# kazuto1011/dusty-gan

Measured on AMD Instinct MI355X. Metric: G+D train images/sec on 64x1024 LiDAR (steps/sec beside it), higher is better.
Workload: dtype bf16

## Files before the change

dusty_gan_amd/_lib.py:

```python
import ctypes as C
import os
import subprocess

_HERE = os.path.dirname(os.path.abspath(__file__))
CSRC = os.path.join(_HERE, "csrc")
LIB_PATH = os.path.join(CSRC, "libdustygan_hip.so")
if os.environ.get("DUSTY_GAN_LIB_DIAG"):
    _d = os.environ["DUSTY_GAN_LIB_DIAG"]
    LIB_PATH = os.path.join(CSRC, "libdustygan_hip_diag%s.so" % ("" if _d == "1" else _d))

DG_OK, DG_EINVAL, DG_EUNSUPPORTED, DG_EHIP = 0, 1, 2, 3
DG_F32, DG_BF16 = 0, 1
DG_BF16X2 = 2
MODE_S2, MODE_UP, MODE_GEMM = 0, 1, 2
EPI_LINEAR, EPI_LRELU, EPI_MASK = 0, 1, 2
DG_FORCE_AUTO, DG_FORCE_DIRECT, DG_FORCE_MFMA, DG_FORCE_THIN, DG_FORCE_LOCKSTEP, DG_FORCE_PINGPONG = 0, 1, 2, 3, 4, 5
DG_FORCE_WG_REGSTAGED, DG_FORCE_WG_DMA_PAIRS, DG_FORCE_WG_DMA_NOPAIRS, DG_FORCE_PINGPONG_SINGLE, DG_FORCE_PROJ_STREAM = 6, 7, 8, 9, 10
DG_FORCE_FP32X3 = 0x100
DG_CONV_FAMILY_DIRECT, DG_CONV_FAMILY_MFMA, DG_CONV_FAMILY_THIN, DG_CONV_FAMILY_LOCKSTEP, DG_CONV_FAMILY_PINGPONG = 1, 2, 3, 4, 5
DG_CONV_FAMILY_PROJ_STREAM = 6
DG_WGRAD_VARIANT_DIRECT, DG_WGRAD_VARIANT_MFMA, DG_WGRAD_VARIANT_THIN, DG_WGRAD_VARIANT_DMA, DG_WGRAD_VARIANT_THIN_MFMA = 1, 2, 3, 5, 7
POLICY_BITS = {"brightness": 1, "saturation": 2, "contrast": 4, "translation": 8, "cutout": 16}

_ERR = {1: "DG_EINVAL (bad argument)", 2: "DG_EUNSUPPORTED (shape not supported by the requested kernel)",
# ... 181 lines not shown
    "dg_transpose_shadow_multi_frags": [_P, _P, _I, _I, _I, C.POINTER(DgUpFrag), _I, _P],
    "dg_transpose_shadow_multi_tail": [_P, _P, _I, _I, _I, C.POINTER(DgUpFrag), _I, _P, _P, _I, _I, _P, _I, _P, _I, _P],
    "dg_philox_bits": [_U64, _U64, _U64, _L, _P, _P],
    "dg_philox_fill": [_U64, _U64, _U64, _I, _F, _F, _I, _I, _L, _P, _P],
    "dg_aug_draw": [_U64, _U64, _U64, _I, _I, _I, _P, _P, _P],
    "dg_counter_add": [_P, _U64, _P],
    "dg_step_prologue": [_P, _P, _I, C.POINTER(DgDraw), _I, _P],
    "dg_step_prologue_fetch": [_P, _P, _I, C.POINTER(DgDraw), _I, C.POINTER(DgFetch), _P],
    "dg_counter_add_multi": [_P, _P, _I, _P],
    "dg_counter_add_multi_snap": [_P, _P, _I, _I, _P, _I, _P, _I, _P],
    "dg_philox_fill_dev": [_U64, _U64, _P, _I, _F, _F, _I, _I, _L, _P, _P],
    "dg_aug_draw_dev": [_U64, _U64, _P, _I, _I, _I, _P, _P, _P],
    "dg_philox_logistic_dev": [_U64, _U64, _P, _F, _L, _P, _P],
    "dg_adam_ema_step_dev": [_P, _P, _P, _P, _P, _P, _I, _L, _F, _F, _F, _F, _F, _P, _F, _P],
    "dg_adam_fused": [_P, _P, _P, _P, _P, _I, C.POINTER(DgOptSeg), _I, _F, _F, _F, _F, _P, _F, _P],
    "dg_adam_proj_fused": [_P, _P, _P, _P, _I, _P, _P, _I, _I, _L, _I, _F, _F, _F, _F, _F, _P, _F, _P],
    "dg_inv_loss_grad": [_P, _L, _I, _P, _P, _P, _I, _I, _L, _F, _P, _I, _P, _I, _P, _P, _I, _P, _P],
    "dg_inv_loss_grad_add": [_P, _L, _I, _P, _P, _P, _I, _I, _L, _F, _P, _I, _P, _I, _P, _P, _I, _P, _P],
    "dg_inv_chamfer_scatter": [_P, _P, _I, _L, _P, _P],
    "dg_inv_chamfer_grad": [_P, _P, _P, _P, _P, _P, _P, _P, _P, _P, _P, _I, _F, _F, _F, _F, _F, _I, _L, _F, _F, _I, _P, _I, _P,
                            _I, _P, _P, _I, _P, _P],
    "dg_sphere_adam": [_P, _L, _L, _P, _P, _P, _P, _P, _P, _P, _I, _I, _I, _P, _I, _F, _F, _F, _I, _U64, _U64, _I, _P],
    "dg_depth_metrics": [_P, _P, _P, _P, _I, _I, _F, _I, _L, _F, _F, _P, _P],
    "dg_feat_compose": [_P, _P, _P, _I, _I, _I, _I, _I, _P],
    "dg_feat_compose_bwd": [_P, _P, _P, _P, _P, _P, _P, _I, _I, _I, _I, _I, _I, _P],
    "dg_alpha_adam": [_P, _P, _P, _P, _P, _P, _I, _F, _F, _F, _L, _P],
    "dg_corrupt_mask": [_P, _P, _P, _P, _F, _I, _I, _I, _P, _P],
    "dg_additive_noise": [_P, _P, _F, _L, _P, _P],
    "dg_median3x3": [_P, _I, _I, _I, _P, _P],
    "dg_hole_fill": [_P, _P, _I, _I, _I, _F, _P, _P, _P],
# ... 287 lines not shown
```

dusty_gan_amd/csrc/optim.hip:

```cpp
#include "adam.h"
#include "step_inputs.h"
#include "thin_up_frag.h"
#include <cstdlib>
typedef __attribute__((ext_vector_type(4))) float f32x4_opt;

template <typename T>
__global__ __launch_bounds__(256) void adam_ema_kernel(float* __restrict__ p, const float* __restrict__ grad,
                                                       float* __restrict__ m, float* __restrict__ v,
                                                       float* __restrict__ ema, T* __restrict__ shadow, long n4,
                                                       float gscale, float lr_bc1, float inv_sqrt_bc2, float b1,
                                                       float b2, float eps, float ema_decay,
                                                       const unsigned long long* __restrict__ stepp, float lr) {
  if (stepp) {
    const float t = adam_step_t(stepp);
    lr_bc1 = adam_lr_bc1(lr, b1, t);
    inv_sqrt_bc2 = adam_inv_sqrt_bc2(b2, t);
  }
  const AdamCoef c{lr_bc1, inv_sqrt_bc2, b2, eps, ema_decay};
  for (long i = (long)blockIdx.x * blockDim.x + threadIdx.x; i < n4; i += (long)gridDim.x * blockDim.x) {
    const float4 g4 = ((const float4*)grad)[i];
    const float4 v4 = ((const float4*)v)[i];
    float4 p4 = ((const float4*)p)[i];
    float4 m4 = m ? ((const float4*)m)[i] : make_float4(0.f, 0.f, 0.f, 0.f);
    float4 e4 = ema ? ((const float4*)ema)[i] : make_float4(0.f, 0.f, 0.f, 0.f);
// ... 5 lines not shown
      mv[k] = b1 * mv[k] + (1.f - b1) * gg[k];
      adam_ema_apply(mv[k], gg[k], vv[k], pv[k], ev[k], c);
    }
    ((float4*)p)[i] = make_float4(pv[0], pv[1], pv[2], pv[3]);
    ((float4*)v)[i] = make_float4(vv[0], vv[1], vv[2], vv[3]);
    if (m) ((float4*)m)[i] = make_float4(mv[0], mv[1], mv[2], mv[3]);
    if (ema) ((float4*)ema)[i] = make_float4(ev[0], ev[1], ev[2], ev[3]);
    if (shadow) shadow_store4(shadow + 4 * i, 0, pv);
  }
}

typedef DgOptSeg OptSeg;
#define OPT_MAX_SEG DG_OPT_MAX_SEG
struct OptSegs { OptSeg s[OPT_MAX_SEG]; int n; int total_blocks; };

template <typename ST>
__global__ __launch_bounds__(256) void adam_fused_kernel(float* __restrict__ p, float* __restrict__ grad, float* __restrict__ v,
                                                         float* __restrict__ ema, ST* __restrict__ shadow, OptSegs segs,
                                                         float gscale, float lr, float b2, float eps, float ema_decay,
                                                         const unsigned long long* __restrict__ stepp) {
  __shared__ f32x4_opt s_part[16][17];
  __shared__ float tile[16 * 65 > 8 * 129 ? 16 * 65 : 8 * 129];
  int k = 0;
  for (int i = 1; i < segs.n; ++i)
    if ((int)blockIdx.x >= segs.s[i].first_block) k = i;
  const OptSeg& sg = segs.s[k];
  const int blk = (int)blockIdx.x - sg.first_block;
  const AdamCoef c{lr, adam_inv_sqrt_bc2(b2, adam_step_t(stepp)), b2, eps, ema_decay};
  struct State { float4 v4, p4, e4; f32x4_opt g0; };
  auto state_load = [&](long i4, bool acc) {
    State st;
    st.v4 = ((const float4*)v)[i4];
    st.p4 = ((const float4*)p)[i4];
    st.e4 = ema ? ((const float4*)ema)[i4] : make_float4(0.f, 0.f, 0.f, 0.f);
    st.g0 = acc ? ((const f32x4_opt*)grad)[i4] : f32x4_opt{0.f, 0.f, 0.f, 0.f};
    return st;
  };
  auto update4 = [&](long i4, f32x4_opt g, const State& st, float (&pn)[4]) {
    const float4 v4 = st.v4, p4 = st.p4, e4 = st.e4;
    ((f32x4_opt*)grad)[i4] = g;
    const float gg[4] = {g[0] * gscale, g[1] * gscale, g[2] * gscale, g[3] * gscale};
    float vv[4] = {v4.x, v4.y, v4.z, v4.w}, ev[4] = {e4.x, e4.y, e4.z, e4.w};
    pn[0] = p4.x; pn[1] = p4.y; pn[2] = p4.z; pn[3] = p4.w;
#pragma unroll
    for (int q = 0; q < 4; ++q) adam_ema_apply(gg[q], gg[q], vv[q], pn[q], ev[q], c);
    ((float4*)p)[i4] = make_float4(pn[0], pn[1], pn[2], pn[3]);
    ((float4*)v)[i4] = make_float4(vv[0], vv[1], vv[2], vv[3]);
    if (ema) ((float4*)ema)[i4] = make_float4(ev[0], ev[1], ev[2], ev[3]);
    if (shadow) shadow_store4(shadow, 4 * i4, pn);
  };
  auto part_sum = [&](long e4, int sp0, int step) {
    f32x4_opt acc = {0.f, 0.f, 0.f, 0.f};
    const f32x4_opt* src = (const f32x4_opt*)sg.part + e4;
    const long stride = sg.numel / 4;
    int sp = sp0;
    for (; sp + 7 * step < sg.splits; sp += 8 * step) {
      f32x4_opt r[8];
#pragma unroll
      for (int j = 0; j < 8; ++j) r[j] = __builtin_nontemporal_load(src + (long)(sp + j * step) * stride);
#pragma unroll
      for (int j = 0; j < 8; ++j) acc += r[j];
// ... 70 lines not shown
  g += st.g0;
  float pn[4];
  update4(i4, g, st, pn);
  float* tl = (float*)tile;
#pragma unroll
  for (int q = 0; q < 4; ++q) tl[ty * (CW + 1) + 4 * tx + q] = pn[q];
  __syncthreads();
  for (int c = threadIdx.x; c < CW; c += 256) {
    ST* dst = (ST*)sg.shadow_t + ((long)tap * Co + co0 + c) * Ci + ci0;
    for (int r0 = 0; r0 < R; r0 += 4) {
      const float o[4] = {tl[(r0 + 0) * (CW + 1) + c], tl[(r0 + 1) * (CW + 1) + c], tl[(r0 + 2) * (CW + 1) + c],
                          tl[(r0 + 3) * (CW + 1) + c]};
      shadow_store4(dst, r0, o);
    }
  }
}

typedef __attribute__((ext_vector_type(2))) __bf16 ad_bf16x2;
#define APF_ROWS 64

template <typename ST>
__global__ __launch_bounds__(256) void adam_proj_fused_kernel(float* __restrict__ p, float* __restrict__ v,
                                                              float* __restrict__ ema, ST* __restrict__ shadow,
                                                              const bf16* __restrict__ dp0, const bf16* __restrict__ zT,
                                                              int nb, long Np, int K, float wscale, float gscale, float lr,
                                                              float b2, float eps, float ema_decay,
                                                              const unsigned long long* __restrict__ stepp) {
  extern __shared__ __attribute__((aligned(16))) unsigned char smem[];
  const int nbp = nb / 2;
  unsigned* z2 = (unsigned*)smem;
// ... 49 lines not shown
  const int tx = threadIdx.x & 31, ty = threadIdx.x >> 5;
  const float* src = master + (long)tap * Ci * Co;
  T* dst = shadow + (long)tap * Ci * Co;
  for (int r = ty; r < 32; r += 8) {
    const int ci = ci0 + r, co = co0 + tx;
    tile[r][tx] = (ci < Ci && co < Co) ? src[(long)ci * Co + co] : 0.f;
  }
  __syncthreads();
  for (int r = ty; r < 32; r += 8) {
    const int co = co0 + r, ci = ci0 + tx;
    if (ci < Ci && co < Co) dst[(long)co * Ci + ci] = (T)tile[tx][r];
  }
}

struct UpFrags { DgUpFrag f[4]; int n; int first_block; };
template <typename T>
__global__ __launch_bounds__(256) void transpose_shadow_multi_kernel(const float* __restrict__ master,
                                                                     const long long* __restrict__ desc, int nseg,
                                                                     UpFrags uf, CounterAdds ca, int ca_block) {
  if ((int)blockIdx.x == ca_block) { counter_adds_body(ca); return; }
  if (uf.n > 0 && (int)blockIdx.x >= uf.first_block) {
    const int job = (int)blockIdx.x - uf.first_block, per = 3 * UP_FRAG_BLOCKS;
    const DgUpFrag& f = uf.f[job / per];
    const int cls = (job % per) / UP_FRAG_BLOCKS, e = ((job % per) % UP_FRAG_BLOCKS) * 256 + threadIdx.x;
    const float* w = master + f.off;
    up_frag_element(cls, e, f.N, f.Hc, f.adj,
                    [&](int tap, int n, int k) { return (float)(bf16)w[tap * f.m_st + n * f.m_sn + k * f.m_sk]; },
                    (unsigned char*)f.frag);
    return;
  }
  int sidx = 0;
  for (int i = 1; i < nseg; ++i)
    if ((long long)blockIdx.x >= desc[5 * i + 4]) sidx = i;
  const long long* d = desc + 5 * sidx;
  const int Ci = (int)d[2], Co = (int)d[3];
  const int tci = (Ci + 31) / 32, tco = (Co + 31) / 32;
  int t = (int)(blockIdx.x - d[4]);
  const int tap = t / (tci * tco);
  t -= tap * tci * tco;
  const int ti = t / tco, tj = t % tco;
  transpose_tile32(master + d[0], (T*)d[1], Ci, Co, tap, ti, tj);
}

template <typename T>
__global__ void cast_kernel(const float* __restrict__ src, T* __restrict__ dst, long n) {
  const long i = (long)blockIdx.x * blockDim.x + threadIdx.x;
  if (i < n) dst[i] = (T)src[i];
}

struct CastItems { const float* src[16]; void* dst[16]; long first8[17]; int n; };
__device__ __forceinline__ void x2_pack8(const float* __restrict__ src, unsigned short* __restrict__ dst, long i8) {
  const float4 a = ((const float4*)src)[2 * i8], b = ((const float4*)src)[2 * i8 + 1];
  const float v[8] = {a.x, a.y, a.z, a.w, b.x, b.y, b.z, b.w};
  unsigned hi[4], lo[4];
#pragma unroll
  for (int e = 0; e < 4; ++e) {
    const bf16 h0 = (bf16)v[2 * e], h1 = (bf16)v[2 * e + 1];
    const bf16 l0 = (bf16)(v[2 * e] - (float)h0), l1 = (bf16)(v[2 * e + 1] - (float)h1);
// ... 113 lines not shown
  if (dtype == DG_BF16) cast_kernel<bf16><<<nblk(n), 256, 0, s>>>(src, (bf16*)dst, n);
  else cast_kernel<float><<<nblk(n), 256, 0, s>>>(src, (float*)dst, n);
  HIP_CHECK_RET(hipGetLastError());
  return DG_OK;
}

int dg_transpose_shadow(const float* master, void* dst, int dtype, int Ci, int Co, void* s_) {
  hipStream_t s = (hipStream_t)s_;
  dim3 grid((Co + 31) / 32, (Ci + 31) / 32, 16);
  if (dtype == DG_BF16) transpose_shadow_kernel<bf16><<<grid, 256, 0, s>>>(master, (bf16*)dst, Ci, Co);
  else transpose_shadow_kernel<float><<<grid, 256, 0, s>>>(master, (float*)dst, Ci, Co);
  HIP_CHECK_RET(hipGetLastError());
  return DG_OK;
}

int dg_adam_fused(float* p, float* grad, float* v, float* ema, void* shadow, int shadow_dtype, const DgOptSeg* segs, int nseg,
                  float gscale, float lr, float beta2, float eps, const unsigned long long* step_dev, float ema_decay, void* s_) {
  hipStream_t s = (hipStream_t)s_;
  if (!p || !grad || !v || !segs || !step_dev || nseg < 1 || nseg > DG_OPT_MAX_SEG) return DG_EINVAL;
  if (shadow && shadow_dtype != DG_BF16 && shadow_dtype != DG_F32) return DG_EINVAL;
  if ((((size_t)p | (size_t)grad | (size_t)v | (size_t)ema | (size_t)shadow) & 15) != 0) return DG_EINVAL;
  OptSegs g{};
  long blocks = 0;
  for (int i = 0; i < nseg; ++i) {
    DgOptSeg q = segs[i];
    if (q.off < 0 || q.numel <= 0 || q.off % 4 != 0 || q.numel % 4 != 0 || q.splits < 0 || (q.splits > 0) != (q.part != nullptr))
      return DG_EINVAL;
    if (q.part && ((size_t)q.part & 15) != 0) return DG_EINVAL;
    if (q.kind == 1) {
      if (q.ci <= 0 || q.co <= 0 || !(q.co == 64 || q.co % 128 == 0) || q.ci % 16 != 0 || q.numel != 16LL * q.ci * q.co ||
          !q.shadow_t || !shadow || ((size_t)q.shadow_t & 15) != 0 || q.ws_src)
        return DG_EINVAL;
      q.first_block = (int)blocks;
      blocks += q.numel / 1024;
    } else if (q.kind == 0) {
      if (q.ws_src && (q.ws_n < 1 || q.ws_stride < q.numel || ((size_t)q.ws_src & 15) != 0 || q.ws_stride % 4 != 0)) return DG_EINVAL;
      if (q.splits > 64) {
        if (q.ws_src) return DG_EINVAL;
        q.kind = 2;
        q.first_block = (int)blocks;
        blocks += (q.numel / 4 + 15) / 16;
      } else {
        q.first_block = (int)blocks;
        blocks += (q.numel / 4 + 255) / 256;
      }
    } else {
      return DG_EINVAL;
    }
    if (blocks > (1L << 30)) return DG_EUNSUPPORTED;
    g.s[i] = q;
  }
  g.n = nseg;
  g.total_blocks = (int)blocks;
  if (shadow && shadow_dtype == DG_BF16)
    adam_fused_kernel<bf16><<<(unsigned)blocks, 256, 0, s>>>(p, grad, v, ema, (bf16*)shadow, g, gscale, lr, beta2, eps, ema_decay, step_dev);
  else
    adam_fused_kernel<float><<<(unsigned)blocks, 256, 0, s>>>(p, grad, v, ema, (float*)shadow, g, gscale, lr, beta2, eps, ema_decay, step_dev);
  HIP_CHECK_RET(hipGetLastError());
  return DG_OK;
}

int dg_adam_proj_fused(float* p, float* v, float* ema, void* shadow, int shadow_dtype, const void* dp0, const void* zT,
                       int op_dtype, int nb, long Np, int K, float wscale, float gscale, float lr, float beta2,
                       float eps, const unsigned long long* step_dev, float ema_decay, void* s_) {
  hipStream_t s = (hipStream_t)s_;
  if (!p || !v || !dp0 || !zT || !step_dev) return DG_EINVAL;
  const int x3 = (op_dtype & DG_FORCE_FP32X3) ? 1 : 0;
  op_dtype &= ~DG_FORCE_FP32X3;
  if ((op_dtype != DG_BF16 && op_dtype != DG_F32) || (x3 && op_dtype != DG_F32) || Np <= 0 || nb < 2) return DG_EUNSUPPORTED;
  const size_t lds = ((size_t)(nb / 2) * K + (size_t)APF_ROWS * (nb / 2)) * 4;
  const bool valu_ok = nb <= 64 && nb % 2 == 0 && K % 4 == 0 && K / 4 <= 256 && 256 % (K / 4) == 0 && lds <= 64 * 1024;
  const bool mfma_ok = Np % 128 == 0 && K % 128 == 0;
  if (op_dtype == DG_F32 && !mfma_ok) return DG_EUNSUPPORTED;
  if (!valu_ok || mfma_ok) {
// ... 67 lines not shown
```

dusty_gan_amd/csrc/step_inputs.h:

```cpp
#pragma once
#include "common.h"

struct CounterAdds {
  unsigned long long* c[8]; unsigned long long d[8]; int k;
  int snap_idx, snap_n, snap_ring; const float* snap_src; float* snap_dst;
};
__device__ __forceinline__ void counter_adds_body(const CounterAdds& a) {
  if ((int)threadIdx.x >= a.k) return;
  const unsigned long long v = *a.c[threadIdx.x];
  *a.c[threadIdx.x] = v + a.d[threadIdx.x];
  if ((int)threadIdx.x == a.snap_idx) {
    float* dst = a.snap_dst + (long)(v % (unsigned long long)a.snap_ring) * a.snap_n;
    for (int i = 0; i < a.snap_n; ++i) dst[i] = a.snap_src[i];
    __threadfence_system();
  }
}
static int fill_counter_adds(CounterAdds& a, unsigned long long* const* counters, const unsigned long long* deltas, int k,
                             int snap_idx, const float* src, int n, float* dst_ring, int ring) {
  if (k < 1 || k > 8 || !counters || !deltas) return DG_EINVAL;
  if (snap_idx >= 0 && (snap_idx >= k || !src || !dst_ring || n < 1 || n > 64 || ring < 1)) return DG_EINVAL;
  a = CounterAdds{};
  a.snap_idx = snap_idx; a.snap_n = n; a.snap_ring = ring; a.snap_src = src; a.snap_dst = dst_ring;
  for (int i = 0; i < k; ++i) {
    if (!counters[i]) return DG_EINVAL;
    for (int j = 0; j < i; ++j)
      if (counters[j] == counters[i]) return DG_EINVAL;
    a.c[i] = counters[i]; a.d[i] = deltas[i];
  }
  a.k = k;
// ... 29 lines not shown
```

dusty_gan_amd/csrc/thin_up_frag.h:

```cpp
#pragma once
#include "common.h"

constexpr int UP_FRAG_BYTES = 3 * 18 * 1024;
constexpr int UP_FRAG_BLOCKS = 36;

template <bool LO = false, typename LoadW>
__device__ __forceinline__ void up_frag_element(int cls, int e, int N, int Hc, int adj, LoadW w, unsigned char* frag) {
  const int m = cls == 0 ? 1 : (cls == 1 ? 0 : Hc - 1);
  if (cls == 0 && Hc < 3) return;
  const int j = e & 7, l = (e >> 3) & 63, f = e >> 9;
  const int half = f & 1, dc = (f >> 1) % 3 - 1, dr = (f >> 1) / 3 - 1;
  const int mp = l & 15, ci = 32 * half + 8 * (l >> 4) + j;
  const int px = mp & 1, q = mp >> 1, py = q / N, n = q % N;
  float v = 0.f;
  if (py < 2) {
    int kx;
    if (px == 0) kx = dc == 0 ? 1 : (dc == -1 ? 3 : -1);
    else kx = dc == 1 ? 0 : (dc == 0 ? 2 : -1);
    if (kx >= 0) {
      for (int i = 0; i < 4; ++i) {
        int r, ky;
        if (dg_tap1d(MODE_UP, adj, 0, 2 * m + py, Hc, i, r, ky) && r - m == dr) v += w(ky * 4 + kx, n, ci);
      }
    }
  }
  *(bf16*)(frag + (((cls * 18 + f) * 64 + l) * 8 + j) * 2) = LO ? (bf16)(v - (float)(bf16)v) : (bf16)v;
}
```

dusty_gan_amd/engine.py:

```python
import ctypes as C
import math
import os
import warnings
from collections import OrderedDict

import torch

from . import _lib as L

ARCH_ID = {"none": 0, "dusty1": 1, "dusty2": 2}

PROFILE = None
TRACE = None


def _align(n, a=64):
    return (n + a - 1) // a * a


class Segment:
    __slots__ = ("name", "off", "shape", "numel", "kind")

    def __init__(self, name, off, shape, kind):
        self.name, self.off, self.shape, self.kind = name, off, tuple(shape), kind
# ... 8 lines not shown
    def __init__(self, segments):
        self.seg = OrderedDict()
        off = 0
        for name, shape, kind in segments:
            s = Segment(name, off, shape, kind)
            self.seg[name] = s
            off = _align(off + s.numel)
        self.n = off
        self.flat = torch.zeros(self.n, dtype=torch.float32)
        self.grad = None
        self.m = None
        self.v = None
        self.shadow = None
        self.coci = {}
        self._tdesc = None
        self.shadow_dtype = None
        self._seen_version = -1
        self.up_frags = {}
        self.x2 = False
        self.x2_cico, self.x2_coci = {}, {}
        self._x2_key = None

    def view(self, name, buf=None):
        s = self.seg[name]
        buf = self.flat if buf is None else buf
        return buf[s.off:s.off + s.numel].view(s.shape)

    def apply(self, fn):
        aliased = self.shadow is self.flat
        self.flat = fn(self.flat)
# ... 114 lines not shown
            desc, tiles = [], 0
            small, stiles = [], 0
            for name, s in convs:
                _, _, ci, co = s.shape
                self.coci[name] = torch.empty(16 * ci * co, dtype=self.shadow_dtype, device=self.flat.device)
                desc += [s.off, L.ptr(self.coci[name]), ci, co, tiles]
                nt = 16 * ((ci + 31) // 32) * ((co + 31) // 32)
                tiles += nt
                if not self.is_fat_conv(name):
                    small += [s.off, L.ptr(self.coci[name]), ci, co, stiles]
                    stiles += nt
            self._tdesc = torch.tensor(desc, dtype=torch.int64).to(self.flat.device)
            self._tdesc_tiles, self._tdesc_dtype = tiles, self.shadow_dtype
            self._tdesc_small = torch.tensor(small, dtype=torch.int64).to(self.flat.device) if small else None
            self._tdesc_small_tiles, self._tdesc_small_n = stiles, len(small) // 5
        tdesc, ntiles, nconv = self._tdesc, self._tdesc_tiles, len(convs)
        if small_only:
            tdesc, ntiles, nconv = self._tdesc_small, self._tdesc_small_tiles, self._tdesc_small_n
        nf = len(self.up_frags) if self.shadow_dtype == torch.bfloat16 else 0
        arr = (L.DgUpFrag * max(nf, 1))(*[d for _, d in self.up_frags.values()][:nf])
        ride = L.Counters.take_for_ride() if tail else None
        if ride is not None:
            L.check(lib.dg_transpose_shadow_multi_tail(L.ptr(self.flat), L.ptr(tdesc), nconv, ntiles,
                                                       L.dtype_code(self.shadow_dtype), arr, nf, *ride, st),
                    "dg_transpose_shadow_multi_tail")
            return
        if nf:
            L.check(lib.dg_transpose_shadow_multi_frags(L.ptr(self.flat), L.ptr(tdesc), nconv, ntiles,
                                                        L.dtype_code(self.shadow_dtype), arr, nf, st),
                    "dg_transpose_shadow_multi_frags")
            return
        if nconv:
            L.check(lib.dg_transpose_shadow_multi(L.ptr(self.flat), L.ptr(tdesc), nconv, ntiles,
                                                  L.dtype_code(self.shadow_dtype), st), "dg_transpose_shadow_multi")

    def sptr(self, name):
        return L.ptr(self.shadow) + self.shadow.element_size() * self.seg[name].off

    def fptr(self, name, buf=None):
        buf = self.flat if buf is None else buf
        return L.ptr(buf) + 4 * self.seg[name].off


def g_segments(nz, ch, shape, nheads):
    h0, w0 = shape[0] >> 4, shape[1] >> 4
    segs = [("proj_w", (h0, w0, ch[3], nz), "gemm"), ("proj_b", (ch[3],), "bias")]
    for i, (ci, co) in enumerate(((ch[3], ch[2]), (ch[2], ch[1]), (ch[1], ch[0])), start=1):
        segs += [(f"up{i}_w", (4, 4, ci, co), "conv"), (f"up{i}_b", (co,), "bias")]
    segs += [("head_w", (4, 4, ch[0], nheads), "conv"), ("head_b", (nheads,), "bias")]
# ... 1125 lines not shown
```

dusty_gan_amd/trainers/dcgan_amp.py:

```python
import math
import os
import os.path as osp
from collections import OrderedDict
from collections.abc import Mapping

import torch
import torch.distributed as dist

from .. import _lib as L
from .. import engine as E
from ..models import define_D, define_G
from ..models.loss import GANLoss
from ..utils import cycle, sigmoid_to_tanh, tanh_to_sigmoid
from ..utils.context_manager import gradient_accumulation
from ..utils import dist as D_
from ..utils.diff_augment import DiffAugment
from ..utils.lidar import LiDAR
from ..utils.rng import Philox
from ..utils.synthetic import SyntheticLiDAR


def _world():
    return dist.get_world_size() if dist.is_available() and dist.is_initialized() else 1

# ... 204 lines not shown
        ses = 2 if shadow_dtype == torch.bfloat16 else 4
        ema_ptr = L.ptr(ema_store.flat) if ema_store is not None else None
        if fused_proj is not None:
            dp0, zT, op_dt, nb, Np, K, wscale = fused_proj
            rc = lib.dg_adam_proj_fused(L.ptr(st.flat), L.ptr(st.v), ema_ptr,
                                        None if st.shadow is st.flat else L.ptr(st.shadow), sdt, L.ptr(dp0), L.ptr(zT),
                                        op_dt, nb, Np, K, wscale, gscale, self.lr, self.betas[1], self.eps,
                                        L.ptr(self._step_dev), ema_decay, L.stream_ptr())
            if rc == L.DG_EUNSUPPORTED:
                return False
            L.check(rc, "dg_adam_proj_fused")
            if between is not None:
                between()
        self.step_count += 1
        self._last_gscale = gscale
        if plan is not None:
            arr, nseg, ws = plan
            L.check(lib.dg_adam_fused(L.ptr(st.flat), L.ptr(st.grad), L.ptr(st.v), ema_ptr, L.ptr(st.shadow), sdt, arr, nseg,
                                      gscale, self.lr, self.betas[1], self.eps, L.ptr(self._step_dev), ema_decay,
                                      L.stream_ptr()), "dg_adam_fused")
            ws.items, ws.pos, ws.demand = [], 0, 0
        else:
            L.check(lib.dg_adam_ema_step_dev(L.ptr(st.flat) + 4 * off, L.ptr(st.grad) + 4 * off,
                                             None if m_ptr is None else m_ptr + 4 * off, L.ptr(st.v) + 4 * off,
                                             None if ema_ptr is None else ema_ptr + 4 * off,
                                             None if st.shadow is st.flat else L.ptr(st.shadow) + ses * off,
                                             sdt, st.n - off, gscale, self.lr, self.betas[0],
                                             self.betas[1], self.eps, L.ptr(self._step_dev), ema_decay, L.stream_ptr()),
                    "dg_adam_ema_step_dev")
        L.Counters.add(self._step_dev, 1)
# ... 996 lines not shown
```

include/dusty_gan_hip.h:

```cpp
#ifndef DUSTY_GAN_HIP_H
#define DUSTY_GAN_HIP_H
#include <stdint.h>

#ifdef __cplusplus
extern "C" {
#endif

#define DG_OK 0
#define DG_EINVAL 1
#define DG_EUNSUPPORTED 2
#define DG_EHIP 3

#define DG_F32 0
#define DG_BF16 1
#define DG_BF16X2 2

#define DG_MODE_S2 0
#define DG_MODE_UP 1
#define DG_MODE_GEMM 2

#define DG_EPI_LINEAR 0
#define DG_EPI_LRELU 1
#define DG_EPI_MASK 2

// ... 310 lines not shown
                         const unsigned long long* step_dev, float ema_decay, void* stream);

#define DG_OPT_MAX_SEG 20
typedef struct DgOptSeg {
  long long off, numel;
  const float* part;
  int splits, accumulate;
  int kind, ci, co;
  void* shadow_t;
  const void* ws_src; const float* ws_coef; long long ws_stride; int ws_n, ws_bf16; float ws_scale;
  int first_block;
} DgOptSeg;
int dg_adam_fused(float* p, float* grad, float* v, float* ema, void* shadow, int shadow_dtype, const DgOptSeg* segs, int nseg,
                  float gscale, float lr, float beta2, float eps, const unsigned long long* step_dev, float ema_decay,
                  void* stream);
int dg_adam_proj_fused(float* p, float* v, float* ema, void* shadow, int shadow_dtype, const void* dp0, const void* zT,
                       int op_dtype, int nb, long Np, int K, float wscale, float gscale, float lr, float beta2,
                       float eps, const unsigned long long* step_dev, float ema_decay, void* stream);

int dg_inv_loss_grad(const float* gen, long gen_sb, int from_tanh, const float* ref, const float* mask, const float* msum,
                     int distance, int B, long HW, float s_depth, float* draw, int nheads, void* draw_pm, int cp,
                     float* parts, unsigned* tickets, int nchunk, float* loss, void* stream);
int dg_inv_loss_grad_add(const float* gen, long gen_sb, int from_tanh, const float* ref, const float* mask, const float* msum,
                         int distance, int B, long HW, float s_depth, float* draw, int nheads, void* draw_pm, int cp,
                         float* parts, unsigned* tickets, int nchunk, float* loss, void* stream);
int dg_inv_chamfer_scatter(const float* R, const int* idx1, int B, long HW, unsigned long long* acc, void* stream);
int dg_inv_chamfer_grad(const float* P, const float* R, const float* d1, const float* d2, const int* idx2,
                        unsigned long long* acc, const float* depth, const float* angle, const float* gout,
                        const float* noise_pixel, const float* mask, int arch, float tau, float drop_const, float min_depth,
                        float max_depth, float tol, int B, long HW, float s_depth, float s_conf, int add, float* draw,
// ... 28 lines not shown
```

Measured before the change: 13760.

## Fuse small-layer shadow transpose, up-frag rebuild and counter adds into Adam kernel tail

Adds an Adam fused kernel variant whose blocks that update the small transposed or up-fragment source parameters publish their results with atomic stores. The last such block, chosen by a ticket, stages the fresh weights in LDS and rebuilds the transposed shadows and up-fragment tables in-kernel. Counter increments ride along through a wave-ticket tail, which removes separate transpose and counter-add launches after the optimizer step. The cost is atomic-store overhead, a single-block serialized tail, and more complex ticket synchronization.

```diff
diff --git a/dusty_gan_amd/_lib.py b/dusty_gan_amd/_lib.py
--- a/dusty_gan_amd/_lib.py
+++ b/dusty_gan_amd/_lib.py
@@ -219,6 +219,8 @@
     "dg_philox_logistic_dev": [_U64, _U64, _P, _F, _L, _P, _P],
     "dg_adam_ema_step_dev": [_P, _P, _P, _P, _P, _P, _I, _L, _F, _F, _F, _F, _F, _P, _F, _P],
     "dg_adam_fused": [_P, _P, _P, _P, _P, _I, C.POINTER(DgOptSeg), _I, _F, _F, _F, _F, _P, _F, _P],
+    "dg_adam_fused_tail": [_P, _P, _P, _P, _P, _I, C.POINTER(DgOptSeg), _I, _F, _F, _F, _F, _P, _F,
+                           _P, _P, _I, C.POINTER(DgUpFrag), _I, _P, _P, _I, _I, _P, _I, _P, _I, _P],
     "dg_adam_proj_fused": [_P, _P, _P, _P, _I, _P, _P, _I, _I, _L, _I, _F, _F, _F, _F, _F, _P, _F, _P],
     "dg_inv_loss_grad": [_P, _L, _I, _P, _P, _P, _I, _I, _L, _F, _P, _I, _P, _I, _P, _P, _I, _P, _P],
     "dg_inv_loss_grad_add": [_P, _L, _I, _P, _P, _P, _I, _I, _L, _F, _P, _I, _P, _I, _P, _P, _I, _P, _P],
diff --git a/dusty_gan_amd/csrc/optim.hip b/dusty_gan_amd/csrc/optim.hip
--- a/dusty_gan_amd/csrc/optim.hip
+++ b/dusty_gan_amd/csrc/optim.hip
@@ -43,18 +43,23 @@
 #define OPT_MAX_SEG DG_OPT_MAX_SEG
 struct OptSegs { OptSeg s[OPT_MAX_SEG]; int n; int total_blocks; };
 
-template <typename ST>
-__global__ __launch_bounds__(256) void adam_fused_kernel(float* __restrict__ p, float* __restrict__ grad, float* __restrict__ v,
-                                                         float* __restrict__ ema, ST* __restrict__ shadow, OptSegs segs,
-                                                         float gscale, float lr, float b2, float eps, float ema_decay,
-                                                         const unsigned long long* __restrict__ stepp) {
-  __shared__ f32x4_opt s_part[16][17];
-  __shared__ float tile[16 * 65 > 8 * 129 ? 16 * 65 : 8 * 129];
-  int k = 0;
-  for (int i = 1; i < segs.n; ++i)
-    if ((int)blockIdx.x >= segs.s[i].first_block) k = i;
-  const OptSeg& sg = segs.s[k];
-  const int blk = (int)blockIdx.x - sg.first_block;
+#define OPT_TAIL_MAX 3072
+#define OPT_LDS_F4 (OPT_TAIL_MAX / 4)
+static_assert(16 * 17 + (16 * 65 > 8 * 129 ? 16 * 65 : 8 * 129) / 4 <= OPT_LDS_F4, "adam_fused_kernel: LDS");
+
+__host__ __device__ inline void opt_block_range(const OptSeg& sg, int blk, long long& b0, long long& b1) {
+  const long long per = sg.kind == 2 ? 64 : 1024;
+  b0 = sg.off + per * blk;
+  b1 = b0 + per < sg.off + sg.numel ? b0 + per : sg.off + sg.numel;
+}
+
+template <typename ST, bool TAIL>
+__device__ __forceinline__ void adam_fused_block(float* __restrict__ p, float* __restrict__ grad, float* __restrict__ v,
+                                                 float* __restrict__ ema, ST* __restrict__ shadow, const OptSeg& sg, const int blk,
+                                                 float gscale, float lr, float b2, float eps, float ema_decay,
+                                                 const unsigned long long* __restrict__ stepp, const bool pub, f32x4_opt* lds) {
+  f32x4_opt (*s_part)[17] = (f32x4_opt (*)[17])lds;
+  float* tile = (float*)(lds + 16 * 17);
   const AdamCoef c{lr, adam_inv_sqrt_bc2(b2, adam_step_t(stepp)), b2, eps, ema_decay};
   struct State { float4 v4, p4, e4; f32x4_opt g0; };
   auto state_load = [&](long i4, bool acc) {
@@ -73,7 +78,12 @@
     pn[0] = p4.x; pn[1] = p4.y; pn[2] = p4.z; pn[3] = p4.w;
 #pragma unroll
     for (int q = 0; q < 4; ++q) adam_ema_apply(gg[q], gg[q], vv[q], pn[q], ev[q], c);
-    ((float4*)p)[i4] = make_float4(pn[0], pn[1], pn[2], pn[3]);
+    if (TAIL && pub) {
+#pragma unroll
+      for (int q = 0; q < 4; ++q) __hip_atomic_store(p + 4 * i4 + q, pn[q], __ATOMIC_RELAXED, __HIP_MEMORY_SCOPE_AGENT);
+    } else {
+      ((float4*)p)[i4] = make_float4(pn[0], pn[1], pn[2], pn[3]);
+    }
     ((float4*)v)[i4] = make_float4(vv[0], vv[1], vv[2], vv[3]);
     if (ema) ((float4*)ema)[i4] = make_float4(ev[0], ev[1], ev[2], ev[3]);
     if (shadow) shadow_store4(shadow, 4 * i4, pn);
@@ -174,6 +184,24 @@
       shadow_store4(dst, r0, o);
     }
   }
+}
+
+__device__ __forceinline__ int opt_seg_of_block(const OptSegs& segs) {
+  int k = 0;
+  for (int i = 1; i < segs.n; ++i)
+    if ((int)blockIdx.x >= segs.s[i].first_block) k = i;
+  return k;
+}
+
+template <typename ST>
+__global__ __launch_bounds__(256) void adam_fused_kernel(float* __restrict__ p, float* __restrict__ grad, float* __restrict__ v,
+                                                         float* __restrict__ ema, ST* __restrict__ shadow, OptSegs segs,
+                                                         float gscale, float lr, float b2, float eps, float ema_decay,
+                                                         const unsigned long long* __restrict__ stepp) {
+  __shared__ f32x4_opt lds[OPT_LDS_F4];
+  const OptSeg& sg = segs.s[opt_seg_of_block(segs)];
+  adam_fused_block<ST, false>(p, grad, v, ema, shadow, sg, (int)blockIdx.x - sg.first_block, gscale, lr, b2, eps, ema_decay, stepp,
+                              false, lds);
 }
 
 typedef __attribute__((ext_vector_type(2))) __bf16 ad_bf16x2;
@@ -253,6 +281,13 @@
 }
 
 struct UpFrags { DgUpFrag f[4]; int n; int first_block; };
+template <typename LoadM>
+__device__ __forceinline__ void up_frag_job(const DgUpFrag& f, int job, LoadM m) {
+  const int cls = job / UP_FRAG_BLOCKS, e = (job % UP_FRAG_BLOCKS) * 256 + threadIdx.x;
+  up_frag_element(cls, e, f.N, f.Hc, f.adj,
+                  [&](int tap, int n, int k) { return (float)(bf16)m(tap * f.m_st + n * f.m_sn + k * f.m_sk); },
+                  (unsigned char*)f.frag);
+}
 template <typename T>
 __global__ __launch_bounds__(256) void transpose_shadow_multi_kernel(const float* __restrict__ master,
                                                                      const long long* __restrict__ desc, int nseg,
@@ -261,11 +296,8 @@
   if (uf.n > 0 && (int)blockIdx.x >= uf.first_block) {
     const int job = (int)blockIdx.x - uf.first_block, per = 3 * UP_FRAG_BLOCKS;
     const DgUpFrag& f = uf.f[job / per];
-    const int cls = (job % per) / UP_FRAG_BLOCKS, e = ((job % per) % UP_FRAG_BLOCKS) * 256 + threadIdx.x;
     const float* w = master + f.off;
-    up_frag_element(cls, e, f.N, f.Hc, f.adj,
-                    [&](int tap, int n, int k) { return (float)(bf16)w[tap * f.m_st + n * f.m_sn + k * f.m_sk]; },
-                    (unsigned char*)f.frag);
+    up_frag_job(f, job % per, [&](long long i) { return w[i]; });
     return;
   }
   int sidx = 0;
@@ -281,6 +313,83 @@
   transpose_tile32(master + d[0], (T*)d[1], Ci, Co, tap, ti, tj);
 }
 
+struct OptTail {
+  unsigned* ticket;
+  int npub, nsrc, ntr, has_ca;
+  unsigned ca_per;
+  long long src_lo[8], src_hi[8];
+  struct { long long off; void* dst; int ci, co; } tr[4];
+  UpFrags uf;
+  CounterAdds ca;
+};
+
+template <typename ST>
+__global__ __launch_bounds__(256) void adam_fused_tail_kernel(float* __restrict__ p, float* __restrict__ grad, float* __restrict__ v,
+                                                              float* __restrict__ ema, ST* __restrict__ shadow, OptSegs segs,
+                                                              float gscale, float lr, float b2, float eps, float ema_decay,
+                                                              const unsigned long long* __restrict__ stepp, OptTail tail) {
+  __shared__ f32x4_opt lds[OPT_LDS_F4];
+  const OptSeg& sg = segs.s[opt_seg_of_block(segs)];
+  const int blk = (int)blockIdx.x - sg.first_block;
+  bool pub = false;
+  if (sg.kind != 1) {
+    long long b0, b1;
+    opt_block_range(sg, blk, b0, b1);
+    for (int i = 0; i < tail.nsrc; ++i) pub |= b0 < tail.src_hi[i] && tail.src_lo[i] < b1;
+  }
+  adam_fused_block<ST, true>(p, grad, v, ema, shadow, sg, blk, gscale, lr, b2, eps, ema_decay, stepp, pub, lds);
+  if (pub) {
+    if (dg_block_ticket_last(tail.ticket, (unsigned)tail.npub)) {
+      if (threadIdx.x == 0) {
+        __builtin_amdgcn_fence(__ATOMIC_ACQUIRE, "agent");
+        asm volatile("s_waitcnt vmcnt(0)" ::: "memory");
+      }
+      __syncthreads();
+      float* cp = (float*)lds;
+      long long have_lo = -1, have_hi = -1;
+      auto stage = [&](long long lo, long long hi) {
+        if (lo == have_lo && hi == have_hi) return;
+        __syncthreads();
+        float r[OPT_TAIL_MAX / 256];
+#pragma unroll
+        for (int u = 0; u < OPT_TAIL_MAX / 256; ++u) {
+          const long long i = threadIdx.x + 256 * u;
+          r[u] = i < hi - lo ? __hip_atomic_load(p + lo + i, __ATOMIC_RELAXED, __HIP_MEMORY_SCOPE_AGENT) : 0.f;
+        }
+#pragma unroll
+        for (int u = 0; u < OPT_TAIL_MAX / 256; ++u) cp[threadIdx.x + 256 * u] = r[u];
+        __syncthreads();
+        have_lo = lo; have_hi = hi;
+      };
+      for (int s = 0; s < tail.ntr; ++s) {
+        const int Ci = tail.tr[s].ci, Co = tail.tr[s].co, n = 16 * Ci * Co;
+        stage(tail.tr[s].off, tail.tr[s].off + n);
+        ST* dst = (ST*)tail.tr[s].dst;
+        for (int e = threadIdx.x; e < n; e += 256) {
+          const int ci = e % Ci, tc = e / Ci, co = tc % Co, tap = tc / Co;
+          dst[e] = (ST)cp[(tap * Ci + ci) * Co + co];
+        }
+      }
+      for (int s = 0; s < tail.uf.n; ++s) {
+        const DgUpFrag& f = tail.uf.f[s];
+        stage(tail.src_lo[tail.ntr + s], tail.src_hi[tail.ntr + s]);
+        up_frag_table(f.N, f.Hc, f.adj,
+                      [&](int tap, int n, int k) { return (float)(bf16)cp[tap * f.m_st + n * f.m_sn + k * f.m_sk]; },
+                      (unsigned char*)f.frag);
+      }
+    }
+  }
+  if (tail.has_ca) {
+    __syncthreads();
+    if (threadIdx.x < 64) {
+      const unsigned grp = blockIdx.x / tail.ca_per, left = gridDim.x - grp * tail.ca_per;
+      if (dg_wave_ticket_last(tail.ticket + 32 * (1 + grp), left < tail.ca_per ? left : tail.ca_per) &&
+          dg_wave_ticket_last(tail.ticket + 1, (gridDim.x + tail.ca_per - 1) / tail.ca_per))
+        counter_adds_body<false>(tail.ca);
+    }
+  }
+}
+
 template <typename T>
 __global__ void cast_kernel(const float* __restrict__ src, T* __restrict__ dst, long n) {
   const long i = (long)blockIdx.x * blockDim.x + threadIdx.x;
@@ -424,14 +533,17 @@
   return DG_OK;
 }
 
-int dg_adam_fused(float* p, float* grad, float* v, float* ema, void* shadow, int shadow_dtype, const DgOptSeg* segs, int nseg,
-                  float gscale, float lr, float beta2, float eps, const unsigned long long* step_dev, float ema_decay, void* s_) {
+static int adam_fused_launch(float* p, float* grad, float* v, float* ema, void* shadow, int shadow_dtype, const DgOptSeg* segs, int nseg,
+                             float gscale, float lr, float beta2, float eps, const unsigned long long* step_dev, float ema_decay,
+                             OptTail* tail, void* s_) {
   hipStream_t s = (hipStream_t)s_;
   if (!p || !grad || !v || !segs || !step_dev || nseg < 1 || nseg > DG_OPT_MAX_SEG) return DG_EINVAL;
   if (shadow && shadow_dtype != DG_BF16 && shadow_dtype != DG_F32) return DG_EINVAL;
   if ((((size_t)p | (size_t)grad | (size_t)v | (size_t)ema | (size_t)shadow) & 15) != 0) return DG_EINVAL;
   OptSegs g{};
-  long blocks = 0;
+  long blocks = 0, nblocks[OPT_MAX_SEG] = {};
+  DgOptSeg in[OPT_MAX_SEG];
+  bool pubseg[OPT_MAX_SEG] = {};
   for (int i = 0; i < nseg; ++i) {
     DgOptSeg q = segs[i];
     if (q.off < 0 || q.numel <= 0 || q.off % 4 != 0 || q.numel % 4 != 0 || q.splits < 0 || (q.splits > 0) != (q.part != nullptr))
@@ -441,33 +553,98 @@
       if (q.ci <= 0 || q.co <= 0 || !(q.co == 64 || q.co % 128 == 0) || q.ci % 16 != 0 || q.numel != 16LL * q.ci * q.co ||
           !q.shadow_t || !shadow || ((size_t)q.shadow_t & 15) != 0 || q.ws_src)
         return DG_EINVAL;
-      q.first_block = (int)blocks;
-      blocks += q.numel / 1024;
+      nblocks[i] = q.numel / 1024;
     } else if (q.kind == 0) {
       if (q.ws_src && (q.ws_n < 1 || q.ws_stride < q.numel || ((size_t)q.ws_src & 15) != 0 || q.ws_stride % 4 != 0)) return DG_EINVAL;
       if (q.splits > 64) {
         if (q.ws_src) return DG_EINVAL;
         q.kind = 2;
-        q.first_block = (int)blocks;
-        blocks += (q.numel / 4 + 15) / 16;
+        nblocks[i] = (q.numel / 4 + 15) / 16;
       } else {
-        q.first_block = (int)blocks;
-        blocks += (q.numel / 4 + 255) / 256;
+        nblocks[i] = (q.numel / 4 + 255) / 256;
       }
     } else {
       return DG_EINVAL;
     }
-    if (blocks > (1L << 30)) return DG_EUNSUPPORTED;
-    g.s[i] = q;
-  }
-  g.n = nseg;
+    if (nblocks[i] > (1L << 30)) return DG_EUNSUPPORTED;
+    if (tail) {
+      for (int r = 0; r < tail->nsrc; ++r) {
+        if (!(q.off < tail->src_hi[r] && tail->src_lo[r] < q.off + q.numel)) continue;
+        if (q.kind == 1) return DG_EINVAL;
+        pubseg[i] = true;
+      }
+      for (long b = 0; pubseg[i] && b < nblocks[i]; ++b) {
+        long long b0, b1;
+        opt_block_range(q, (int)b, b0, b1);
+        bool pub = false;
+        for (int r = 0; r < tail->nsrc; ++r) pub |= b0 < tail->src_hi[r] && tail->src_lo[r] < b1;
+        tail->npub += pub ? 1 : 0;
+      }
+    }
+    in[i] = q;
+  }
+  for (int pass = 0; pass < 2; ++pass)
+    for (int i = 0; i < nseg; ++i) {
+      if (pubseg[i] != (pass == 0)) continue;
+      in[i].first_block = (int)blocks;
+      blocks += nblocks[i];
+      if (blocks > (1L << 30)) return DG_EUNSUPPORTED;
+      g.s[g.n++] = in[i];
+    }
   g.total_blocks = (int)blocks;
-  if (shadow && shadow_dtype == DG_BF16)
+  if (tail) {
+    if (tail->npub < 1) return DG_EINVAL;
+    tail->ca_per = (unsigned)((blocks + 63) / 64);
+    if (shadow && shadow_dtype == DG_BF16)
+      adam_fused_tail_kernel<bf16><<<(unsigned)blocks, 256, 0, s>>>(p, grad, v, ema, (bf16*)shadow, g, gscale, lr, beta2, eps, ema_decay, step_dev, *tail);
+    else
+      adam_fused_tail_kernel<float><<<(unsigned)blocks, 256, 0, s>>>(p, grad, v, ema, (float*)shadow, g, gscale, lr, beta2, eps, ema_decay, step_dev, *tail);
+  } else if (shadow && shadow_dtype == DG_BF16)
     adam_fused_kernel<bf16><<<(unsigned)blocks, 256, 0, s>>>(p, grad, v, ema, (bf16*)shadow, g, gscale, lr, beta2, eps, ema_decay, step_dev);
   else
     adam_fused_kernel<float><<<(unsigned)blocks, 256, 0, s>>>(p, grad, v, ema, (float*)shadow, g, gscale, lr, beta2, eps, ema_decay, step_dev);
   HIP_CHECK_RET(hipGetLastError());
   return DG_OK;
+}
+int dg_adam_fused(float* p, float* grad, float* v, float* ema, void* shadow, int shadow_dtype, const DgOptSeg* segs, int nseg,
+                  float gscale, float lr, float beta2, float eps, const unsigned long long* step_dev, float ema_decay, void* s_) {
+  return adam_fused_launch(p, grad, v, ema, shadow, shadow_dtype, segs, nseg, gscale, lr, beta2, eps, step_dev, ema_decay, nullptr, s_);
+}
+int dg_adam_fused_tail(float* p, float* grad, float* v, float* ema, void* shadow, int shadow_dtype, const DgOptSeg* segs, int nseg,
+                       float gscale, float lr, float beta2, float eps, const unsigned long long* step_dev, float ema_decay,
+                       unsigned* ticket, const long long* desc, int ntr, const DgUpFrag* frags, int nfrag,
+                       unsigned long long* const* counters, const unsigned long long* deltas, int k, int snap_idx, const float* src,
+                       int n, float* dst_ring, int ring, void* s_) {
+  if (!ticket || ((size_t)ticket & 127) || ntr < 0 || ntr > 4 || nfrag < 0 || nfrag > 4 || (ntr && !desc) || (nfrag && !frags) ||
+      ntr + nfrag < 1 || !shadow)
+    return DG_EINVAL;
+  if (nfrag && shadow_dtype != DG_BF16) return DG_EUNSUPPORTED;
+  OptTail t{};
+  t.ticket = ticket;
+  t.ntr = ntr;
+  for (int i = 0; i < ntr; ++i) {
+    const long long* d = desc + 5 * i;
+    if (d[0] < 0 || !d[1] || d[2] < 1 || d[3] < 1 || 16 * d[2] * d[3] > OPT_TAIL_MAX) return DG_EUNSUPPORTED;
+    t.tr[i].off = d[0]; t.tr[i].dst = (void*)d[1]; t.tr[i].ci = (int)d[2]; t.tr[i].co = (int)d[3];
+    t.src_lo[i] = d[0]; t.src_hi[i] = d[0] + 16 * d[2] * d[3];
+  }
+  t.uf.n = nfrag;
+  for (int i = 0; i < nfrag; ++i) {
+    const DgUpFrag& f = frags[i];
+    if (!f.frag || ((size_t)f.frag & 15) || f.N < 1 || f.N > 4 || f.Hc < 1 || f.off < 0 || f.m_st < 0 || f.m_sn < 0 || f.m_sk < 0)
+      return DG_EINVAL;
+    const long long span = 15 * f.m_st + (f.N - 1) * f.m_sn + 63 * f.m_sk + 1;
+    if (span > OPT_TAIL_MAX) return DG_EUNSUPPORTED;
+    t.uf.f[i] = f;
+    t.src_lo[ntr + i] = f.off; t.src_hi[ntr + i] = f.off + span;
+  }
+  t.nsrc = ntr + nfrag;
+  if (k > 0) {
+    const int rc = fill_counter_adds(t.ca, counters, deltas, k, snap_idx, src, n, dst_ring, ring);
+    if (rc != DG_OK) return rc;
+    t.has_ca = 1;
+  }
+  return adam_fused_launch(p, grad, v, ema, shadow, shadow_dtype, segs, nseg, gscale, lr, beta2, eps, step_dev, ema_decay, &t, s_);
 }
 
 int dg_adam_proj_fused(float* p, float* v, float* ema, void* shadow, int shadow_dtype, const void* dp0, const void* zT,
diff --git a/dusty_gan_amd/csrc/step_inputs.h b/dusty_gan_amd/csrc/step_inputs.h
--- a/dusty_gan_amd/csrc/step_inputs.h
+++ b/dusty_gan_amd/csrc/step_inputs.h
@@ -5,6 +5,7 @@
   unsigned long long* c[8]; unsigned long long d[8]; int k;
   int snap_idx, snap_n, snap_ring; const float* snap_src; float* snap_dst;
 };
+template <bool FENCE = true>
 __device__ __forceinline__ void counter_adds_body(const CounterAdds& a) {
   if ((int)threadIdx.x >= a.k) return;
   const unsigned long long v = *a.c[threadIdx.x];
@@ -12,7 +13,7 @@
   if ((int)threadIdx.x == a.snap_idx) {
     float* dst = a.snap_dst + (long)(v % (unsigned long long)a.snap_ring) * a.snap_n;
     for (int i = 0; i < a.snap_n; ++i) dst[i] = a.snap_src[i];
-    __threadfence_system();
+    if (FENCE) __threadfence_system();
   }
 }
 static int fill_counter_adds(CounterAdds& a, unsigned long long* const* counters, const unsigned long long* deltas, int k,
diff --git a/dusty_gan_amd/csrc/thin_up_frag.h b/dusty_gan_amd/csrc/thin_up_frag.h
--- a/dusty_gan_amd/csrc/thin_up_frag.h
+++ b/dusty_gan_amd/csrc/thin_up_frag.h
@@ -4,25 +4,59 @@
 constexpr int UP_FRAG_BYTES = 3 * 18 * 1024;
 constexpr int UP_FRAG_BLOCKS = 36;
 
+__device__ __forceinline__ void up_frag_taps(int cls, int f, int mp, int N, int Hc, int adj, int (&tap)[4], int& n) {
+  const int m = cls == 0 ? 1 : (cls == 1 ? 0 : Hc - 1);
+  const int dc = (f >> 1) % 3 - 1, dr = (f >> 1) / 3 - 1;
+  const int px = mp & 1, q = mp >> 1, py = q / N;
+  n = q % N;
+  int kx;
+  if (px == 0) kx = dc == 0 ? 1 : (dc == -1 ? 3 : -1);
+  else kx = dc == 1 ? 0 : (dc == 0 ? 2 : -1);
+#pragma unroll
+  for (int i = 0; i < 4; ++i) {
+    int r = 0, ky = 0;
+    const bool on = py < 2 && kx >= 0 && dg_tap1d(MODE_UP, adj, 0, 2 * m + py, Hc, i, r, ky) && r - m == dr;
+    tap[i] = on ? ky * 4 + kx : -1;
+  }
+}
+template <typename LoadW>
+__device__ __forceinline__ float up_frag_sum(const int (&tap)[4], int n, int ci, LoadW w) {
+  float x[4];
+#pragma unroll
+  for (int i = 0; i < 4; ++i) x[i] = w(tap[i] >= 0 ? tap[i] : 0, n, ci);
+  float v = 0.f;
+#pragma unroll
+  for (int i = 0; i < 4; ++i) v += tap[i] >= 0 ? x[i] : 0.f;
+  return v;
+}
+
 template <bool LO = false, typename LoadW>
 __device__ __forceinline__ void up_frag_element(int cls, int e, int N, int Hc, int adj, LoadW w, unsigned char* frag) {
-  const int m = cls == 0 ? 1 : (cls == 1 ? 0 : Hc - 1);
   if (cls == 0 && Hc < 3) return;
   const int j = e & 7, l = (e >> 3) & 63, f = e >> 9;
-  const int half = f & 1, dc = (f >> 1) % 3 - 1, dr = (f >> 1) / 3 - 1;
-  const int mp = l & 15, ci = 32 * half + 8 * (l >> 4) + j;
-  const int px = mp & 1, q = mp >> 1, py = q / N, n = q % N;
-  float v = 0.f;
-  if (py < 2) {
-    int kx;
-    if (px == 0) kx = dc == 0 ? 1 : (dc == -1 ? 3 : -1);
-    else kx = dc == 1 ? 0 : (dc == 0 ? 2 : -1);
-    if (kx >= 0) {
-      for (int i = 0; i < 4; ++i) {
-        int r, ky;
-        if (dg_tap1d(MODE_UP, adj, 0, 2 * m + py, Hc, i, r, ky) && r - m == dr) v += w(ky * 4 + kx, n, ci);
+  const int ci = 32 * (f & 1) + 8 * (l >> 4) + j;
+  int tap[4], n;
+  up_frag_taps(cls, f, l & 15, N, Hc, adj, tap, n);
+  const float v = up_frag_sum(tap, n, ci, w);
+  *(bf16*)(frag + (((cls * 18 + f) * 64 + l) * 8 + j) * 2) = LO ? (bf16)(v - (float)(bf16)v) : (bf16)v;
+}
+template <typename LoadW>
+__device__ __forceinline__ void up_frag_table(int N, int Hc, int adj, LoadW w, unsigned char* frag) {
+  for (int c = threadIdx.x; c < 3 * 18 * 16; c += 256) {
+    const int cls = c / (18 * 16), f = (c / 16) % 18, mp = c & 15;
+    if (cls == 0 && Hc < 3) continue;
+    int tap[4], n;
+    up_frag_taps(cls, f, mp, N, Hc, adj, tap, n);
+#pragma unroll
+    for (int g = 0; g < 4; ++g) {
+      unsigned pk[4];
+#pragma unroll
+      for (int j2 = 0; j2 < 4; ++j2) {
+        const int ci = 32 * (f & 1) + 8 * g + 2 * j2;
+        const bf16 a = (bf16)up_frag_sum(tap, n, ci, w), b = (bf16)up_frag_sum(tap, n, ci + 1, w);
+        pk[j2] = (unsigned)__builtin_bit_cast(unsigned short, a) | ((unsigned)__builtin_bit_cast(unsigned short, b) << 16);
       }
+      *(uint4*)(frag + ((cls * 18 + f) * 64 + mp + 16 * g) * 16) = make_uint4(pk[0], pk[1], pk[2], pk[3]);
     }
   }
-  *(bf16*)(frag + (((cls * 18 + f) * 64 + l) * 8 + j) * 2) = LO ? (bf16)(v - (float)(bf16)v) : (bf16)v;
 }
diff --git a/dusty_gan_amd/engine.py b/dusty_gan_amd/engine.py
--- a/dusty_gan_amd/engine.py
+++ b/dusty_gan_amd/engine.py
@@ -46,6 +46,7 @@
         self.shadow = None
         self.coci = {}
         self._tdesc = None
+        self._opt_ticket = None
         self.shadow_dtype = None
         self._seen_version = -1
         self.up_frags = {}
@@ -190,6 +191,7 @@
             self._tdesc_tiles, self._tdesc_dtype = tiles, self.shadow_dtype
             self._tdesc_small = torch.tensor(small, dtype=torch.int64).to(self.flat.device) if small else None
             self._tdesc_small_tiles, self._tdesc_small_n = stiles, len(small) // 5
+            self._tdesc_small_host = (C.c_longlong * max(len(small), 1))(*small)
         tdesc, ntiles, nconv = self._tdesc, self._tdesc_tiles, len(convs)
         if small_only:
             tdesc, ntiles, nconv = self._tdesc_small, self._tdesc_small_tiles, self._tdesc_small_n
@@ -209,6 +211,29 @@
         if nconv:
             L.check(lib.dg_transpose_shadow_multi(L.ptr(self.flat), L.ptr(tdesc), nconv, ntiles,
                                                   L.dtype_code(self.shadow_dtype), st), "dg_transpose_shadow_multi")
+
+    opt_tail_enabled = os.environ.get("DUSTY_GAN_OPT_TAIL", "1") != "0"
+    opt_tail_ride = os.environ.get("DUSTY_GAN_OPT_TAIL", "1") == "2"
+    OPT_TAIL_MAX = 3072
+
+    def opt_tail(self, off):
+        if not ParamStore.opt_tail_enabled or self._tdesc is None or self._tdesc_dtype != self.shadow_dtype or self.x2:
+            return None
+        if self._tdesc.device != self.flat.device or self.shadow_dtype != torch.bfloat16:
+            return None
+        ntr, d = self._tdesc_small_n, self._tdesc_small_host
+        fr = [f for _, f in self.up_frags.values()]
+        if ntr > 4 or ntr + len(fr) < 1:
+            return None
+        for i in range(ntr):
+            if d[5 * i] < off or 16 * d[5 * i + 2] * d[5 * i + 3] > self.OPT_TAIL_MAX:
+                return None
+        for f in fr:
+            if f.off < off or 15 * f.m_st + (f.N - 1) * f.m_sn + 63 * f.m_sk + 1 > self.OPT_TAIL_MAX:
+                return None
+        if self._opt_ticket is None or self._opt_ticket.device != self.flat.device:
+            self._opt_ticket = torch.zeros(65 * 32, dtype=torch.int32, device=self.flat.device)
+        return L.ptr(self._opt_ticket), d, ntr, (L.DgUpFrag * max(len(fr), 1))(*fr), len(fr)
 
     def sptr(self, name):
         return L.ptr(self.shadow) + self.shadow.element_size() * self.seg[name].off
diff --git a/dusty_gan_amd/trainers/dcgan_amp.py b/dusty_gan_amd/trainers/dcgan_amp.py
--- a/dusty_gan_amd/trainers/dcgan_amp.py
+++ b/dusty_gan_amd/trainers/dcgan_amp.py
@@ -242,6 +242,18 @@
                 between()
         self.step_count += 1
         self._last_gscale = gscale
+        tail = st.opt_tail(off) if plan is not None and (E.ParamStore.opt_tail_ride or not L.Counters.ride) else None
+        if tail is not None:
+            arr, nseg, ws = plan
+            L.Counters.add(self._step_dev, 1)
+            ride = L.Counters.take_for_ride() or (None, None, 0, -1, None, 0, None, 1)
+            L.check(lib.dg_adam_fused_tail(L.ptr(st.flat), L.ptr(st.grad), L.ptr(st.v), ema_ptr, L.ptr(st.shadow), sdt, arr, nseg,
+                                           gscale, self.lr, self.betas[1], self.eps, L.ptr(self._step_dev), ema_decay,
+                                           *tail, *ride, L.stream_ptr()), "dg_adam_fused_tail")
+            ws.items, ws.pos, ws.demand = [], 0, 0
+            if ema_store is not None:
+                ema_store._seen_version = -1
+            return True
         if plan is not None:
             arr, nseg, ws = plan
             L.check(lib.dg_adam_fused(L.ptr(st.flat), L.ptr(st.grad), L.ptr(st.v), ema_ptr, L.ptr(st.shadow), sdt, arr, nseg,
diff --git a/include/dusty_gan_hip.h b/include/dusty_gan_hip.h
--- a/include/dusty_gan_hip.h
+++ b/include/dusty_gan_hip.h
@@ -348,6 +348,11 @@
 int dg_adam_fused(float* p, float* grad, float* v, float* ema, void* shadow, int shadow_dtype, const DgOptSeg* segs, int nseg,
                   float gscale, float lr, float beta2, float eps, const unsigned long long* step_dev, float ema_decay,
                   void* stream);
+int dg_adam_fused_tail(float* p, float* grad, float* v, float* ema, void* shadow, int shadow_dtype, const DgOptSeg* segs, int nseg,
+                       float gscale, float lr, float beta2, float eps, const unsigned long long* step_dev, float ema_decay,
+                       unsigned* ticket, const long long* desc, int ntr, const DgUpFrag* frags, int nfrag,
+                       unsigned long long* const* counters, const unsigned long long* deltas, int k, int snap_idx,
+                       const float* src, int n, float* dst_ring, int ring, void* stream);
 int dg_adam_proj_fused(float* p, float* v, float* ema, void* shadow, int shadow_dtype, const void* dp0, const void* zT,
                        int op_dtype, int nb, long Np, int K, float wscale, float gscale, float lr, float beta2,
                        float eps, const unsigned long long* step_dev, float ema_decay, void* stream);
```

Measured after the change: 13750. About the same (-0.0%).
